# tsurumeso/vocal-remover

Hardware: NVIDIA H100
Metric: seconds-of-audio/sec separated (n_fft=2048, hop=1024) (higher is better)
Workload: dtype bf16x3 (split-bf16 operands hi+lo, 3 wgmma passes, fp32 accumulate); fft/lstm fp32

## Files before the change

### vocal-remover_b200/csrc/api.cu

```cuda
#include <stdio.h>
#include <string.h>

#include <string>

#include "../../include/vr_b200.h"
#include "engine.h"
#include "kernels.h"
#include "tc_plan.h"

struct vr_ctx {
  vr::Engine* eng;
  std::string err;
};

static std::string g_create_err;

static int fail(vr_ctx* c, const std::string& m) {
  (c ? c->err : g_create_err) = m;
  return -1;
}
static void use_device(const vr_ctx* c) {
  if (c && c->eng) cudaSetDevice(c->eng->cfg().device);
}
static int done(vr_ctx* c, bool ok) {
// ... 330 lines not shown
  if (e != cudaSuccess) return fail(ctx, std::string("vr_shared_alloc: cudaMalloc: ") + cudaGetErrorString(e));
  cudaIpcMemHandle_t h;
  e = cudaIpcGetMemHandle(&h, p);
  if (e != cudaSuccess) {
    cudaFree(p);
    return fail(ctx, std::string("vr_shared_alloc: cudaIpcGetMemHandle: ") + cudaGetErrorString(e));
  }
  memcpy(handle64, &h, 64);
  *dev_ptr = p;
  return 0;
}

int vr_shared_open(vr_ctx* ctx, const unsigned char* handle64, void** dev_ptr) {
  CHECK_CTX(ctx);
  if (!dev_ptr || !handle64) return fail(ctx, "vr_shared_open: bad arguments");
  cudaIpcMemHandle_t h;
  memcpy(&h, handle64, 64);
  void* p = nullptr;
  cudaError_t e = cudaIpcOpenMemHandle(&p, h, cudaIpcMemLazyEnablePeerAccess);
  if (e != cudaSuccess) return fail(ctx, std::string("vr_shared_open: cudaIpcOpenMemHandle: ") + cudaGetErrorString(e));
  *dev_ptr = p;
  return 0;
}

int vr_shared_close(vr_ctx* ctx, void* dev_ptr, int32_t owner) {
  CHECK_CTX(ctx);
  if (!dev_ptr) return 0;
  cudaError_t e = owner ? cudaFree(dev_ptr) : cudaIpcCloseMemHandle(dev_ptr);
  if (e != cudaSuccess) return fail(ctx, std::string("vr_shared_close: ") + cudaGetErrorString(e));
  return 0;
}

int64_t vr_launch_count(const vr_ctx* ctx) { return ctx && ctx->eng ? ctx->eng->launches : 0; }

int vr_profile_enable(vr_ctx* ctx, int32_t on) {
  CHECK_CTX(ctx);
  ctx->eng->profile_enable(on != 0);
  return 0;
}

int vr_profile_read(vr_ctx* ctx, double* out6) {
  CHECK_CTX(ctx);
  return done(ctx, ctx->eng->profile_read(out6));
}

int vr_profile_dump(vr_ctx* ctx, char* text, int64_t cap, int64_t* needed) {
  CHECK_CTX(ctx);
  std::string t;
  if (!ctx->eng->profile_dump(t)) return done(ctx, false);
  if (needed) *needed = (int64_t)t.size() + 1;
  if (text && cap > 0) {
    const size_t n = t.size() < (size_t)cap - 1 ? t.size() : (size_t)cap - 1;
    memcpy(text, t.data(), n);
    text[n] = 0;
  }
  return 0;
}

int vr_debug_conv(vr_ctx* ctx, const float* x, int32_t N, int32_t Cin, int32_t H, int32_t W, const float* w,
                  const float* bias, int32_t Cout, int32_t k, int32_t stride, int32_t dil_h, int32_t dil_w, int32_t act,
                  int32_t use_tc, float* y, void* stream) {
  CHECK_CTX(ctx);
  return done(ctx, ctx->eng->debug_conv(x, N, Cin, H, W, w, bias, Cout, k, stride, dil_h, dil_w, act, use_tc, y,
                                        (cudaStream_t)stream));
}

int vr_debug_decoder(vr_ctx* ctx, const float* low, int32_t N, int32_t Cl, int32_t h, int32_t w, const float* skip,
                     int32_t Cs, const float* wgt, const float* bias, int32_t Cout, int32_t act, int32_t fused, float* y,
                     void* stream) {
  CHECK_CTX(ctx);
  return done(ctx, ctx->eng->debug_decoder(low, N, Cl, h, w, skip, Cs, wgt, bias, Cout, act, fused, y,
                                           (cudaStream_t)stream));
}

int vr_debug_tensor(vr_ctx* ctx, const char* name, int32_t n0, int32_t n, float* out, int64_t* shape4, void* stream) {
  CHECK_NET(ctx);
  if (!name || !shape4) return fail(ctx, "vr_debug_tensor: name and shape4 are required");
  return done(ctx, ctx->eng->debug_tensor(name, n0, n, out, shape4, (cudaStream_t)stream));
}

int vr_debug_set(int32_t key, int32_t value) {
  int* knob = key == 0 ? &vr::g_debug.trace : key == 2 ? &vr::g_debug.rows_wide : key == 3 ? &vr::g_debug.halo
            : key == 6 ? &vr::g_debug.kskip : key == 7 ? &vr::g_debug.crop_mask
            : key == 8 ? &vr::g_debug.pair : key == 9 ? &vr::g_debug.pair_stores : nullptr;
  if (!knob) return -1;
  *knob = value;
  return 0;
}

int64_t vr_debug_trace(uint64_t* host_out, int64_t capacity) {
  return vr::tc_rows_read_trace((unsigned long long*)host_out, (long long)capacity);
}

}
```

### vocal-remover_b200/csrc/conv_tc_rows.cu

```cuda
#include <stdio.h>

#include "engine.h"
#include "tc_common.cuh"
#include "tc_plan.h"

namespace vr {

static constexpr int kInterpWarps = 10;
static constexpr int kConsumerWarps = 8;
static constexpr int kTmaWarp = kConsumerWarps;
static constexpr int kInterpWarp0 = kConsumerWarps + 1;
__host__ __device__ constexpr int rows_per_tile(int BN) { return BN == 64 ? 2 : BN == 32 ? 4 : 8; }
static constexpr int kUpProducerWarps = 12;
static constexpr int kUpConsumerRegs = 128;
static constexpr int kUpProducerRegs = 72;
static constexpr int kUpLaunchRegs = 96;
static_assert(kConsumerWarps * kUpConsumerRegs + kUpProducerWarps * kUpProducerRegs <=
                  (kConsumerWarps + kUpProducerWarps) * kUpLaunchRegs,
              "setmaxnreg.inc would wait forever for registers the block does not own");
__host__ __device__ constexpr int rows_threads(bool up) { return 32 * (kConsumerWarps + (up ? kUpProducerWarps : 1)); }
static constexpr int kRowPx = 130;
static constexpr int kBoxPx = 136;
static constexpr int kMaxASlots = 8;
static constexpr int kStaticSmem = 3072;
static constexpr int kSrcPx = 68;
static constexpr uint32_t kKB = 32;
static constexpr uint32_t kRowB = kKB * 2;
static constexpr uint32_t kAPlane = kBoxPx * kRowB;
static constexpr uint32_t kASlot = 2 * kAPlane;

static constexpr int kTraceEvents = 2048;
__device__ unsigned long long g_rows_trace[3 * kTraceEvents * 3];

template <int BN>
struct RowsGeom {
  static constexpr uint32_t kBPlane = 3 * BN * kRowB;
  static constexpr uint32_t kBKw = 2 * kBPlane;
  static constexpr uint32_t kBBuf = 3 * kBKw;
};

struct RowsParams {
  int N, H, W, tiles_w, tiles_h, n_tiles, total_tiles;
  int col0;
  int chunks, CinPadR, Cout, act;
  int n_aslots;
  bf16* out_hi;
  bf16* out_lo;
  int64_t osn, osh;
  int osw;
  int vec16;
  const float* bias;
  int up_chunks, xH, xW;
  const bf16* x_hi;
  const bf16* x_lo;
  int64_t xsn, xsh;
  int xsw;
  int trace;
  unsigned long long kmask;
  int a_c_off;
  int l_chunk;
  int n_uslots;
  float up_sh, up_sw;
  const float* dot_w;
  float* dot_out;
  MaskOutParams mask;
};

struct RowsTile {
  int nt, w0, h0, n;
};
template <int R>
__device__ __forceinline__ RowsTile rows_tile(const RowsParams& p, int tile) {
  RowsTile t;
  t.nt = tile % p.n_tiles;
  int mt = tile / p.n_tiles;
  t.w0 = p.col0 + (mt % p.tiles_w) * 128;
  mt /= p.tiles_w;
  t.h0 = (mt % p.tiles_h) * R;
  t.n = mt / p.tiles_h;
  return t;
}

struct RowsConsumer {
  MbarRing a_up, a_tma, b;
  HeldSlot held_b;
};

template <int BN, int R, int r>
__device__ __forceinline__ MbarRing consume_rows(MbarRing a, RowsConsumer& st, float* acc, uint32_t (&fr)[2][16],
                                                 uint32_t lrow, uint32_t bsrc, uint32_t dhi, uint32_t ksm, int lane) {
  constexpr int o_lo = r - 2 < 0 ? 0 : r - 2;
  constexpr int o_hi = r > R - 1 ? R - 1 : r;
  a.wait_full();
  const uint32_t row = lrow + (uint32_t)a.slot * kASlot;
#pragma unroll
  for (int kw = 0; kw < 3; ++kw) {
    uint32_t* f = fr[(3 * r + kw) & 1];
    const uint32_t q = (row >> 6) + (uint32_t)kw;
#pragma unroll
    for (int ks = 0; ks < 2; ++ks) {
      if (!((ksm >> ks) & 1u)) continue;
      const uint32_t a = (q << 6) + ((((uint32_t)(2 * ks) + ((uint32_t)lane >> 4)) ^ ((q >> 1) & 3u)) << 4);
      ldsm_x4(f + 8 * ks, a);
      ldsm_x4(f + 8 * ks + 4, a + kAPlane);
    }
    wg_fence();
#pragma unroll
    for (int ks = 0; ks < 2; ++ks) {
      if (!((ksm >> ks) & 1u)) continue;
      const uint32_t bo = (uint32_t)(kw * RowsGeom<BN>::kBKw + ks * 32) >> 4;
#pragma unroll
      for (int o = o_lo; o <= o_hi; ++o) {
        const uint32_t b_row = bsrc + (((uint32_t)((2 - (r - o)) * BN) * kRowB) >> 4) + bo;
        wgmma_split3_rs<BN>(acc + o * (BN / 2), f + 8 * ks, f + 8 * ks + 4, b_row,
                            b_row + (RowsGeom<BN>::kBPlane >> 4), dhi);
      }
    }
    wg_commit();
    if (kw == 2) warp_arrive(a.empty(), lane);
    wg_wait<1>();
    st.held_b.release(st.b, lane);
  }
  a.advance();
  if constexpr (r + 1 < R + 2)
    return consume_rows<BN, R, r + 1>(a, st, acc, fr, lrow, bsrc, dhi, ksm, lane);
  else
    return a;
}

__device__ __forceinline__ float dot_pair(float v0, float v1, const float* bias_s, const float* dot_s, int c, float slope) {
  const float t0 = v0 + bias_s[c], t1 = v1 + bias_s[c + 1];
  return fmaf(fmaxf(t0, 0.f) + slope * fminf(t0, 0.f), dot_s[c], (fmaxf(t1, 0.f) + slope * fminf(t1, 0.f)) * dot_s[c + 1]);
}

template <int BN>
__device__ __forceinline__ void mask_pixel(const RowsParams& p, const float* v, const float* bias_s,
                                           const float* mask_s, float slope, int lane, int n, int bin, int w) {
  float x[BN / 4];
#pragma unroll
  for (int j = 0; j < BN / 8; ++j) {
    const int c = 8 * j + 2 * (lane & 3);
    const float t0 = v[4 * j] + bias_s[c], t1 = v[4 * j + 1] + bias_s[c + 1];
    const float y0 = fmaxf(t0, 0.f) + slope * fminf(t0, 0.f);
    const float y1 = fmaxf(t1, 0.f) + slope * fminf(t1, 0.f);
    const float2 hf = bf2_to_f2(f2_to_bf2(y0, y1));
    const float2 lf = bf2_to_f2(f2_to_bf2(y0 - hf.x, y1 - hf.y));
    x[2 * j] = hf.x + lf.x;
    x[2 * j + 1] = hf.y + lf.y;
  }
  const float* wm = mask_s + (lane & 1) * BN;
  float a = 0.f;
#pragma unroll
  for (int c = 0; c < BN; ++c)
    a = fmaf(__shfl_sync(0xffffffffu, x[2 * (c >> 3) + (c & 1)], (lane & ~3) | ((c >> 1) & 3)), wm[c], a);
  const float m = 1.f / (1.f + expf(-a));
  const int tr = w - p.col0;
  const int64_t t = p.mask.t_base0 + (int64_t)n * p.mask.roi_t + tr;
  const bool nyquist = (lane & 2) != 0;
  if (t < 0 || t >= p.mask.t_limit || (nyquist && bin != p.H - 1)) return;
  float* d = p.mask.out + (int64_t)n * p.mask.stride_n + (int64_t)(nyquist ? bin + 1 : bin) * p.mask.stride_bin +
             p.mask.t_base0 + tr + ((lane & 1) ? p.mask.stride_c : 0);
  *d = p.mask.accumulate ? (*d + m) * 0.5f : m;
}

template <int BN, bool UP>
__global__ void __launch_bounds__(rows_threads(UP), 1)
    conv_tc_rows_kernel(const __grid_constant__ CUtensorMap tmA, const __grid_constant__ CUtensorMap tmB,
                        const __grid_constant__ CUtensorMap tmL, const RowsParams p) {
  typedef RowsGeom<BN> G;
  constexpr int R = rows_per_tile(BN);
  extern __shared__ uint8_t smem_raw[];
  __shared__ __align__(8) uint64_t bar_afull[kMaxASlots];
  __shared__ __align__(8) uint64_t bar_aempty[kMaxASlots];
  __shared__ __align__(8) uint64_t bar_bfull[2];
  __shared__ __align__(8) uint64_t bar_bempty[2];
  __shared__ float bias_s[256];
  __shared__ float dot_s[256];

  const int warp = __shfl_sync(0xffffffffu, (int)threadIdx.x >> 5, 0);
  const int lane = threadIdx.x & 31;
  const uint32_t smem_base = (smem_u32(smem_raw) + 1023u) & ~1023u;
  const uint32_t a_base = smem_base;
  const uint32_t b_base = smem_base + (uint32_t)p.n_aslots * kASlot;
  MbarRing a_up(smem_u32(&bar_afull[0]), smem_u32(&bar_aempty[0]), 0, p.n_uslots);
  MbarRing a_tma(smem_u32(&bar_afull[0]), smem_u32(&bar_aempty[0]), p.n_uslots, p.n_aslots);
  MbarRing b_ring(smem_u32(&bar_bfull[0]), smem_u32(&bar_bempty[0]), 0, 2);

  if (warp == kTmaWarp && lane == 0) {
    tma_prefetch(&tmA);
    tma_prefetch(&tmB);
    a_up.init(kInterpWarps, kConsumerWarps);
    a_tma.init(1, kConsumerWarps);
    b_ring.init(1, kConsumerWarps);
    asm volatile("fence.mbarrier_init.release.cluster;" ::: "memory");
  }
  for (int i = threadIdx.x; i < p.n_tiles * BN; i += blockDim.x) {
    bias_s[i] = __ldg(p.bias + i);
    dot_s[i] = p.dot_out && i < p.Cout ? __ldg(p.dot_w + i) : 0.f;
  }
  constexpr bool kMaskable = UP && BN <= 32;
  if constexpr (kMaskable) {
    if (p.mask.out)
      for (int i = threadIdx.x; i < 2 * BN; i += blockDim.x) dot_s[i] = __ldg(p.mask.w + i);
  }
  __syncthreads();
  if (warp < kConsumerWarps) {
    if constexpr (UP) setmaxnreg_inc<kUpConsumerRegs>();
    const int wg = warp >> 2;
    const float slope = act_slope(p.act);
    const uint32_t dhi = desc_hi(8 * kRowB, 2u);
    const uint32_t lrow = a_base + (uint32_t)(64 * wg + 16 * (warp & 3) + (lane & 15)) * kRowB;
    RowsConsumer st{a_up, a_tma, b_ring};
    float acc[R * BN / 2];
    uint32_t fr[2][16];
    for (int tile = blockIdx.x; tile < p.total_tiles; tile += gridDim.x) {
#pragma unroll
      for (int i = 0; i < R * BN / 2; ++i) acc[i] = 0.f;
      for (int cc = 0; cc < p.chunks; ++cc) {
        st.b.wait_full();
        const uint32_t bsrc = desc_lo(b_base + (uint32_t)st.b.slot * G::kBBuf);
        const bool up = cc < p.up_chunks;
        const uint32_t gm = chunk_groups(p.kmask, cc);
        const uint32_t ksm = ((gm & 0x3u) ? 1u : 0u) | ((gm & 0xCu) ? 2u : 0u);
        const MbarRing a = consume_rows<BN, R, 0>(up ? st.a_up : st.a_tma, st, acc, fr, lrow, bsrc, dhi, ksm, lane);
        st.a_up.slot = up ? a.slot : st.a_up.slot;
        st.a_up.phase = up ? a.phase : st.a_up.phase;
        st.a_tma.slot = up ? st.a_tma.slot : a.slot;
        st.a_tma.phase = up ? st.a_tma.phase : a.phase;
        st.held_b.hold(st.b);
        st.b.advance();
      }
      wg_wait<0>();
      st.held_b.release_last(st.b, lane);

      const RowsTile tl = rows_tile<R>(p, tile);
      const int w0 = tl.w0, h0 = tl.h0, n = tl.n;
      const int c_lane = tl.nt * BN + 2 * (lane & 3);
      auto dot = [&](const float* v, int orow, int px) {
        float d = 0.f;
#pragma unroll
        for (int j = 0; j < BN / 8; ++j) d += dot_pair(v[4 * j], v[4 * j + 1], bias_s, dot_s, c_lane + 8 * j, slope);
        d += __shfl_xor_sync(0xffffffffu, d, 1);
        d += __shfl_xor_sync(0xffffffffu, d, 2);
        if ((lane & 3) == 0) atomicAdd(p.dot_out + ((int64_t)n * p.H + (h0 + orow)) * p.W + (w0 + px), d);
      };
      const int px0 = 64 * wg + 16 * (warp & 3) + (lane >> 2);
#pragma unroll
      for (int orow = 0; orow < R; ++orow) {
        if constexpr (UP) {
          constexpr bool kPixel8 = BN > 16;
#pragma unroll
          for (int hr = 0; hr < 2; ++hr) {
            const int px = px0 + 8 * hr;
            const float* v = acc + orow * (BN / 2) + 2 * hr;
            if constexpr (kMaskable) {
              if (p.mask.out) {
                mask_pixel<BN>(p, v, bias_s, dot_s, slope, lane, n, h0 + orow, w0 + px);
                continue;
              }
            }
            if (p.dot_out) dot(v, orow, px);
            const int64_t obase = (int64_t)n * p.osn + (int64_t)(h0 + orow) * p.osh + (int64_t)(w0 + px) * p.osw;
            epilogue_pixel8<BN>(v, bias_s, tl.nt * BN, p.Cout, slope, lane, p.out_hi + obase, p.out_lo + obase,
                                kPixel8 && p.vec16 != 0);
          }
        } else {
          const float* v = acc + orow * (BN / 2);
          if (p.dot_out) {
            dot(v, orow, px0);
            dot(v + 2, orow, px0 + 8);
          }
          const int64_t obase = (int64_t)n * p.osn + (int64_t)(h0 + orow) * p.osh + (int64_t)(w0 + px0) * p.osw;
          const EpiDest d{p.out_hi, p.out_lo, {obase, obase + 8 * (int64_t)p.osw}, {true, true}, tl.nt * BN, p.Cout,
                          p.vec16 != 0};
          epilogue_store<BN>(v, bias_s, slope, lane, d);
        }
      }
    }
  } else {
    if constexpr (UP) setmaxnreg_dec<kUpProducerRegs>();
    if (warp == kTmaWarp) {
      if (elect_one_sync()) {
#ifdef VR_TRACE
        const bool tr = p.trace && blockIdx.x == 0;
#else
        constexpr bool tr = false;
#endif
        int tn = 0;
        for (int tile = blockIdx.x; tile < p.total_tiles; tile += gridDim.x) {
          const RowsTile tl = rows_tile<R>(p, tile);
          const int nt = tl.nt, w0 = tl.w0, h0 = tl.h0, n = tl.n;
          for (int cc = 0; cc < p.chunks; ++cc) {
            b_ring.wait_empty();
            const uint32_t bdst = b_base + (uint32_t)b_ring.slot * G::kBBuf;
            mbar_expect_tx(b_ring.full(), G::kBBuf);
#pragma unroll
            for (int kw = 0; kw < 3; ++kw)
              tma_load_3d(bdst + (uint32_t)kw * G::kBKw, &tmB, kw * p.CinPadR + cc * (int)kKB, nt * 3 * BN, 0,
                          b_ring.full());
            b_ring.advance();
            if (cc < p.up_chunks) continue;
            const bool from_l = cc == p.l_chunk;
            const int c0 = from_l ? 0 : cc * (int)kKB + p.a_c_off;
            for (int r = 0; r < R + 2; ++r) {
              const unsigned long long t0 = tr ? clock64() : 0ull;
              a_tma.wait_empty();
              mbar_expect_tx(a_tma.full(), kASlot);
              tma_load_5d(a_base + (uint32_t)a_tma.slot * kASlot, from_l ? &tmL : &tmA, c0, w0 - 1, h0 - 1 + r, n, 0,
                          a_tma.full());
              if (tr && tn < kTraceEvents) {
                g_rows_trace[(1 * kTraceEvents + tn) * 3 + 0] = t0;
                g_rows_trace[(1 * kTraceEvents + tn) * 3 + 1] = clock64();
                g_rows_trace[(1 * kTraceEvents + tn) * 3 + 2] = 0ull;
                ++tn;
              }
              a_tma.advance();
            }
          }
        }
      }
      __syncwarp();
    } else if (UP && warp < kInterpWarp0 + kInterpWarps) {
      if (p.up_chunks > 0) {
        const int wk = warp - kInterpWarp0;
        const int xi = lane >> 2, j = lane & 3;
        const int sx = 7 * wk + xi;
        const bool emit = xi < 7 && sx < kSrcPx;
        const float inv_sw = p.up_sw > 0.f ? 1.f / p.up_sw : 0.f;
#ifdef VR_TRACE
        const bool tr = p.trace && blockIdx.x == 0 && wk == 0;
#else
        constexpr bool tr = false;
#endif
        int tn = 0;
        const int my_tiles = (p.total_tiles - (int)blockIdx.x + (int)gridDim.x - 1) / (int)gridDim.x;
        const int fills = my_tiles * p.up_chunks * (R + 2);
        int f_tile = blockIdx.x, f_cc = 0, f_r = 0, f_h0 = 0, f_X = 0;
        int64_t f_base = 0;
        bool f_px = false;
        auto fetch_tile = [&]() {
          const RowsTile tl = rows_tile<R>(p, f_tile);
          f_h0 = tl.h0 - 1;
          f_X = (int)(p.up_sw * (tl.w0 > 0 ? tl.w0 - 1 : 0)) + sx;
          f_px = sx < kSrcPx && f_X < p.xW;
          f_base = (int64_t)tl.n * p.xsn + (int64_t)f_X * p.xsw + j * 8;
        };
        fetch_tile();
        bf16x8 qah, qch, qal, qcl, nah, nch, nal, ncl;
        float q_ly = 0.f, n_ly = 0.f;
        qah = qch = qal = qcl = nah = nch = nal = ncl = make_uint4(0, 0, 0, 0);
        auto fetch = [&]() {
          qah = nah; qch = nch; qal = nal; qcl = ncl;
          q_ly = n_ly;
          const int h = f_h0 + f_r;
          const bool grp = (chunk_groups(p.kmask, f_cc) >> j) & 1u;
          if (f_tile < p.total_tiles && h >= 0 && h < p.H && grp && f_px) {
            const float fy = p.up_sh * h;
            const int y0 = (int)fy;
            n_ly = fy - (float)y0;
            const int64_t o0 = f_base + (int64_t)y0 * p.xsh + f_cc * 32;
            const int64_t o1 = o0 + (y0 < p.xH - 1 ? p.xsh : 0);
// ... 98 lines not shown
            }
          }
        }
      }
      }
  }
}

#define VR_ROWS_FOR_ALL(X) X(16, true) X(16, false) X(32, true) X(32, false) X(64, true) X(64, false)

static int rows_b_bytes(int BN) {
#define VR_ROWS_B(BN_, UP_) if (BN == BN_) return (int)(2 * RowsGeom<BN_>::kBBuf);
  VR_ROWS_FOR_ALL(VR_ROWS_B)
#undef VR_ROWS_B
  return 0;
}

bool tc_rows_has(int BN) { return rows_b_bytes(BN) > 0; }

cudaError_t tc_rows_launch(const ConvLayer& L, TcConv& tc, const ActView& in, const ActView& out, cudaStream_t s,
                           std::string& err, const ConvFusion& f) {
  const ActView* up_src = f.up;
  if (up_src && (!tc.fuses_upsample(up_src->C) || up_src->H * 2 != in.H || up_src->W * 2 != in.W || up_src->sw % 8)) {
    err = "tc_rows_launch: fused upsample needs a half-resolution source of 32k channels";
    return cudaErrorInvalidValue;
  }
  if (up_src && up_src->C + in.C > tc.CinPad) {
    err = "tc_rows_launch: with a fused upsample the input must hold only the channels after the up-sampled ones";
    return cudaErrorInvalidValue;
  }
  const ActView* last = f.last_chunk;
  if (last && (last->H != in.H || last->W != in.W || last->N != in.N || last->C > tc.KB)) {
    err = "tc_rows_launch: the last-chunk tensor must match the input geometry and fit one chunk";
    return cudaErrorInvalidValue;
  }
  const CUtensorMap* map_a = tc_activation_map(tc, in, kBoxPx, 1, 1, 1, err, L.name);
  const CUtensorMap* map_l = last ? tc_activation_map(tc, *last, kBoxPx, 1, 1, 1, err, L.name) : map_a;
  if (!map_a || !map_l) return cudaErrorInvalidValue;
  if (f.mask && !tc.fuses_mask(L.Cout, f.mask->offset, up_src != nullptr)) {
    err = "tc_rows_launch: the fused output layer needs a fused upsample, one N tile of Cout <= 32 channels and a "
          "kept width that is a multiple of 128";
    return cudaErrorInvalidValue;
  }
  const int col0 = f.mask ? f.mask->offset : 0;
  RowsParams p;
  p.N = out.N; p.H = out.H; p.W = out.W;
  const bool up = up_src != nullptr;
  p.col0 = col0;
  p.tiles_w = (out.W - 2 * col0) / 128; p.tiles_h = out.H / rows_per_tile(tc.BN); p.n_tiles = tc.n_tiles;
  p.total_tiles = p.tiles_w * p.tiles_h * out.N * tc.n_tiles;
  p.chunks = tc.chunks; p.CinPadR = tc.CinPad; p.Cout = L.Cout; p.act = L.act;
  p.out_hi = out.hi; p.out_lo = out.lo;
  p.osn = out.sn; p.osh = out.sh; p.osw = out.sw;
  p.vec16 = tc_vec16(out);
  p.bias = tc.bias.get();
  p.up_chunks = 0; p.xH = p.xW = 0;
  p.x_hi = p.x_lo = nullptr; p.xsn = p.xsh = 0; p.xsw = 0;
  p.trace = g_debug.trace == 1 ? 1 : 0;
  p.up_sh = p.up_sw = 0.f;
  p.dot_w = f.dot_w; p.dot_out = f.dot_w ? f.dot_out : nullptr;
  p.mask = f.mask ? *f.mask : MaskOutParams{};
  p.a_c_off = 0;
  p.l_chunk = last ? tc.chunks - 1 : -1;
  p.kmask = g_debug.kskip == 1 ? tc.kmask : ~0ull;
  if (up_src) {
    p.a_c_off = -up_src->C;
    p.up_chunks = up_src->C / 32;
    p.xH = up_src->H; p.xW = up_src->W;
    p.x_hi = up_src->hi; p.x_lo = up_src->lo;
    p.xsn = up_src->sn; p.xsh = up_src->sh; p.xsw = up_src->sw;
    if ((reinterpret_cast<uintptr_t>(up_src->hi) | reinterpret_cast<uintptr_t>(up_src->lo)) & 15) {
      err = "tc_rows_launch: upsample source planes must be 16-byte aligned";
      return cudaErrorInvalidValue;
    }
    p.up_sh = in.H > 1 ? (float)(up_src->H - 1) / (float)(in.H - 1) : 0.f;
    p.up_sw = in.W > 1 ? (float)(up_src->W - 1) / (float)(in.W - 1) : 0.f;
  }
  const TcDevice& dv = tc_device();
  if (!dv.ok) {
    err = "tc_rows_launch: cannot query the current device";
    return cudaErrorInvalidValue;
  }
  const int b_bytes = rows_b_bytes(tc.BN);
  p.n_aslots = (dv.max_smem - kStaticSmem - 1024 - b_bytes) / (int)kASlot;
  if (p.n_aslots > kMaxASlots) p.n_aslots = kMaxASlots;
  if (p.n_aslots < (p.up_chunks > 0 ? 4 : 2)) {
    err = "tc_rows_launch: shared memory too small";
    return cudaErrorInvalidValue;
  }
  p.n_uslots = p.up_chunks > 0 ? p.n_aslots - p.n_aslots / 2 : 0;
  if (p.up_chunks > 0 && p.n_aslots - p.n_uslots < 2) p.n_uslots = p.n_aslots - 2;
  const int dyn = p.n_aslots * (int)kASlot + b_bytes + 1024;
  const int grid = p.total_tiles < dv.num_sms ? p.total_tiles : dv.num_sms;
  const int threads = rows_threads(up);
#define VR_ROWS_LAUNCH(BN_, UP_)                                                              \
  if (tc.BN == BN_ && up == UP_) {                                                            \
    conv_tc_rows_kernel<BN_, UP_><<<grid, threads, dyn, s>>>(*map_a, tc.map_b, *map_l, p);    \
    return cudaGetLastError();                                                                \
  }
  VR_ROWS_FOR_ALL(VR_ROWS_LAUNCH)
#undef VR_ROWS_LAUNCH
  err = "tc_rows_launch: no kernel instantiation for this channel tile";
  return cudaErrorInvalidValue;
}


int tc_rows_read_trace(unsigned long long* out, long long capacity) {
  const long long n = 3LL * kTraceEvents * 3;
  if (capacity < n) return -1;
  if (cudaMemcpyFromSymbol(out, g_rows_trace, sizeof(unsigned long long) * (size_t)n) != cudaSuccess) return -1;
  return (int)n;
}

void tc_rows_set_attributes(int max_smem) {
#define VR_ROWS_SET(BN_, UP_)                                                                        \
  cudaFuncSetAttribute(conv_tc_rows_kernel<BN_, UP_>, cudaFuncAttributeMaxDynamicSharedMemorySize,   \
                       max_smem - kStaticSmem);                                                      \
  cudaFuncSetAttribute(conv_tc_rows_kernel<BN_, UP_>, cudaFuncAttributePreferredSharedMemoryCarveout, 100);
  VR_ROWS_FOR_ALL(VR_ROWS_SET)
#undef VR_ROWS_SET
}

}
```

### vocal-remover_b200/csrc/tc_common.cuh

```cuda
#pragma once
#include <cuda.h>
#include <stdint.h>
#include <stdio.h>

#include "common.cuh"

namespace vr {

__device__ __forceinline__ uint32_t smem_u32(const void* p) { return (uint32_t)__cvta_generic_to_shared(p); }

__device__ __forceinline__ bool elect_one_sync() {
  uint32_t pred;
  asm volatile(
      "{\n\t"
      ".reg .pred P1;\n\t"
      "elect.sync _|P1, 0xffffffff;\n\t"
      "selp.u32 %0, 1, 0, P1;\n\t"
      "}"
      : "=r"(pred));
  return pred != 0;
}

__device__ __forceinline__ void mbar_init(uint32_t bar, uint32_t count) {
  asm volatile("mbarrier.init.shared::cta.b64 [%0], %1;" ::"r"(bar), "r"(count));
// ... 21 lines not shown
      "WAIT_DONE:\n\t"
      "}" ::"r"(bar),
      "r"(parity)
      : "memory");
#else
  asm volatile(
      "{\n\t"
      ".reg .pred p;\n\t"
      "WAIT_LOOP:\n\t"
      "mbarrier.try_wait.parity.shared::cta.b64 p, [%0], %1;\n\t"
      "@p bra WAIT_DONE;\n\t"
      "bra WAIT_LOOP;\n\t"
      "WAIT_DONE:\n\t"
      "}" ::"r"(bar),
      "r"(parity)
      : "memory");
#endif
}
__device__ __forceinline__ void warp_arrive(uint32_t bar, int lane) {
  __syncwarp();
  if (lane == 0) mbar_arrive(bar);
}

struct MbarRing {
  uint32_t full0, empty0;
  int lo, hi, slot;
  uint32_t phase;

  __device__ __forceinline__ MbarRing(uint32_t full0_, uint32_t empty0_, int lo_, int hi_)
      : full0(full0_), empty0(empty0_), lo(lo_), hi(hi_), slot(lo_), phase(0) {}
  __device__ __forceinline__ uint32_t full(int s) const { return full0 + (uint32_t)s * 8u; }
  __device__ __forceinline__ uint32_t empty(int s) const { return empty0 + (uint32_t)s * 8u; }
  __device__ __forceinline__ uint32_t full() const { return full(slot); }
  __device__ __forceinline__ uint32_t empty() const { return empty(slot); }
  __device__ __forceinline__ void wait_full() const { mbar_wait(full(), phase); }
  __device__ __forceinline__ void wait_empty() const { mbar_wait(empty(), phase ^ 1u); }
  __device__ __forceinline__ void advance() {
    if (++slot == hi) {
      slot = lo;
      phase ^= 1u;
    }
  }
  __device__ __forceinline__ void init(uint32_t full_count, uint32_t empty_count) const {
    for (int s = lo; s < hi; ++s) {
      mbar_init(full(s), full_count);
      mbar_init(empty(s), empty_count);
    }
  }
};

struct HeldSlot {
  int slot = -1;
  __device__ __forceinline__ void hold(const MbarRing& r) { slot = r.slot; }
  __device__ __forceinline__ void release(const MbarRing& r, int lane) {
    if (slot >= 0) {
      warp_arrive(r.empty(slot), lane);
      slot = -1;
    }
  }
  __device__ __forceinline__ void release_last(const MbarRing& r, int lane) {
    warp_arrive(r.empty(slot), lane);
    slot = -1;
  }
};

__device__ __forceinline__ void tma_prefetch(const CUtensorMap* map) {
  asm volatile("prefetch.tensormap [%0];" ::"l"(map) : "memory");
}
__device__ __forceinline__ void tma_load_5d(uint32_t dst, const CUtensorMap* map, int c0, int c1, int c2, int c3,
                                            int c4, uint32_t bar) {
  asm volatile(
      "cp.async.bulk.tensor.5d.shared::cluster.global.tile.mbarrier::complete_tx::bytes [%0], [%1, {%2, %3, %4, %5, "
      "%6}], [%7];" ::"r"(dst),
      "l"(map), "r"(c0), "r"(c1), "r"(c2), "r"(c3), "r"(c4), "r"(bar)
      : "memory");
}
__device__ __forceinline__ void tma_load_3d(uint32_t dst, const CUtensorMap* map, int c0, int c1, int c2,
                                            uint32_t bar) {
  asm volatile(
      "cp.async.bulk.tensor.3d.shared::cluster.global.tile.mbarrier::complete_tx::bytes [%0], [%1, {%2, %3, %4}], "
      "[%5];" ::"r"(dst),
      "l"(map), "r"(c0), "r"(c1), "r"(c2), "r"(bar)
      : "memory");
}

__device__ __forceinline__ uint32_t desc_lo(uint32_t addr) { return ((addr & 0x3FFFFu) >> 4) | (1u << 16); }
__device__ __forceinline__ uint32_t desc_hi(uint32_t sbo_bytes, uint32_t layout_type) {
  return (sbo_bytes >> 4) | (layout_type << 30);
}
__device__ __forceinline__ uint64_t desc64(uint32_t lo, uint32_t hi) { return ((uint64_t)hi << 32) | lo; }

__device__ __forceinline__ void wg_fence() { asm volatile("wgmma.fence.sync.aligned;" ::: "memory"); }
__device__ __forceinline__ void wg_commit() { asm volatile("wgmma.commit_group.sync.aligned;" ::: "memory"); }
template <int PENDING>
__device__ __forceinline__ void wg_wait() {
  asm volatile("wgmma.wait_group.sync.aligned %0;" ::"n"(PENDING) : "memory");
}

template <int N>
struct Wgmma;
template <>
struct Wgmma<16> {
  static __device__ __forceinline__ void mma(float* d, uint64_t a, uint64_t b) {
    asm volatile(
        "wgmma.mma_async.sync.aligned.m64n16k16.f32.bf16.bf16 {%0, %1, %2, %3, %4, %5, %6, %7}, %8, %9, 1, 1, 1, 0, 0;"
        : "+f"(d[0]), "+f"(d[1]), "+f"(d[2]), "+f"(d[3]), "+f"(d[4]), "+f"(d[5]), "+f"(d[6]), "+f"(d[7])
        : "l"(a), "l"(b)
        : "memory");
  }
};
template <>
struct Wgmma<32> {
  static __device__ __forceinline__ void mma(float* d, uint64_t a, uint64_t b) {
    asm volatile(
        "wgmma.mma_async.sync.aligned.m64n32k16.f32.bf16.bf16 {%0, %1, %2, %3, %4, %5, %6, %7, %8, %9, %10, %11, %12, %13, %14, %15}, %16, %17, 1, 1, 1, 0, 0;"
        : "+f"(d[0]), "+f"(d[1]), "+f"(d[2]), "+f"(d[3]), "+f"(d[4]), "+f"(d[5]), "+f"(d[6]), "+f"(d[7]), "+f"(d[8]), "+f"(d[9]), "+f"(d[10]), "+f"(d[11]), "+f"(d[12]), "+f"(d[13]), "+f"(d[14]), "+f"(d[15])
        : "l"(a), "l"(b)
        : "memory");
  }
};
template <>
struct Wgmma<48> {
  static __device__ __forceinline__ void mma(float* d, uint64_t a, uint64_t b) {
    asm volatile(
        "wgmma.mma_async.sync.aligned.m64n48k16.f32.bf16.bf16 {%0, %1, %2, %3, %4, %5, %6, %7, %8, %9, %10, %11, %12, %13, %14, %15, %16, %17, %18, %19, %20, %21, %22, %23}, %24, %25, 1, 1, 1, 0, 0;"
        : "+f"(d[0]), "+f"(d[1]), "+f"(d[2]), "+f"(d[3]), "+f"(d[4]), "+f"(d[5]), "+f"(d[6]), "+f"(d[7]), "+f"(d[8]), "+f"(d[9]), "+f"(d[10]), "+f"(d[11]), "+f"(d[12]), "+f"(d[13]), "+f"(d[14]), "+f"(d[15]), "+f"(d[16]), "+f"(d[17]), "+f"(d[18]), "+f"(d[19]), "+f"(d[20]), "+f"(d[21]), "+f"(d[22]), "+f"(d[23])
        : "l"(a), "l"(b)
        : "memory");
  }
};
template <>
struct Wgmma<64> {
  static __device__ __forceinline__ void mma(float* d, uint64_t a, uint64_t b) {
    asm volatile(
        "wgmma.mma_async.sync.aligned.m64n64k16.f32.bf16.bf16 {%0, %1, %2, %3, %4, %5, %6, %7, %8, %9, %10, %11, %12, %13, %14, %15, %16, %17, %18, %19, %20, %21, %22, %23, %24, %25, %26, %27, %28, %29, %30, %31}, %32, %33, 1, 1, 1, 0, 0;"
        : "+f"(d[0]), "+f"(d[1]), "+f"(d[2]), "+f"(d[3]), "+f"(d[4]), "+f"(d[5]), "+f"(d[6]), "+f"(d[7]), "+f"(d[8]), "+f"(d[9]), "+f"(d[10]), "+f"(d[11]), "+f"(d[12]), "+f"(d[13]), "+f"(d[14]), "+f"(d[15]), "+f"(d[16]), "+f"(d[17]), "+f"(d[18]), "+f"(d[19]), "+f"(d[20]), "+f"(d[21]), "+f"(d[22]), "+f"(d[23]), "+f"(d[24]), "+f"(d[25]), "+f"(d[26]), "+f"(d[27]), "+f"(d[28]), "+f"(d[29]), "+f"(d[30]), "+f"(d[31])
        : "l"(a), "l"(b)
        : "memory");
  }
};
template <>
struct Wgmma<80> {
  static __device__ __forceinline__ void mma(float* d, uint64_t a, uint64_t b) {
    asm volatile(
        "wgmma.mma_async.sync.aligned.m64n80k16.f32.bf16.bf16 {%0, %1, %2, %3, %4, %5, %6, %7, %8, %9, %10, %11, %12, %13, %14, %15, %16, %17, %18, %19, %20, %21, %22, %23, %24, %25, %26, %27, %28, %29, %30, %31, %32, %33, %34, %35, %36, %37, %38, %39}, %40, %41, 1, 1, 1, 0, 0;"
        : "+f"(d[0]), "+f"(d[1]), "+f"(d[2]), "+f"(d[3]), "+f"(d[4]), "+f"(d[5]), "+f"(d[6]), "+f"(d[7]), "+f"(d[8]), "+f"(d[9]), "+f"(d[10]), "+f"(d[11]), "+f"(d[12]), "+f"(d[13]), "+f"(d[14]), "+f"(d[15]), "+f"(d[16]), "+f"(d[17]), "+f"(d[18]), "+f"(d[19]), "+f"(d[20]), "+f"(d[21]), "+f"(d[22]), "+f"(d[23]), "+f"(d[24]), "+f"(d[25]), "+f"(d[26]), "+f"(d[27]), "+f"(d[28]), "+f"(d[29]), "+f"(d[30]), "+f"(d[31]), "+f"(d[32]), "+f"(d[33]), "+f"(d[34]), "+f"(d[35]), "+f"(d[36]), "+f"(d[37]), "+f"(d[38]), "+f"(d[39])
        : "l"(a), "l"(b)
        : "memory");
  }
};
template <>
struct Wgmma<96> {
  static __device__ __forceinline__ void mma(float* d, uint64_t a, uint64_t b) {
    asm volatile(
        "wgmma.mma_async.sync.aligned.m64n96k16.f32.bf16.bf16 {%0, %1, %2, %3, %4, %5, %6, %7, %8, %9, %10, %11, %12, %13, %14, %15, %16, %17, %18, %19, %20, %21, %22, %23, %24, %25, %26, %27, %28, %29, %30, %31, %32, %33, %34, %35, %36, %37, %38, %39, %40, %41, %42, %43, %44, %45, %46, %47}, %48, %49, 1, 1, 1, 0, 0;"
        : "+f"(d[0]), "+f"(d[1]), "+f"(d[2]), "+f"(d[3]), "+f"(d[4]), "+f"(d[5]), "+f"(d[6]), "+f"(d[7]), "+f"(d[8]), "+f"(d[9]), "+f"(d[10]), "+f"(d[11]), "+f"(d[12]), "+f"(d[13]), "+f"(d[14]), "+f"(d[15]), "+f"(d[16]), "+f"(d[17]), "+f"(d[18]), "+f"(d[19]), "+f"(d[20]), "+f"(d[21]), "+f"(d[22]), "+f"(d[23]), "+f"(d[24]), "+f"(d[25]), "+f"(d[26]), "+f"(d[27]), "+f"(d[28]), "+f"(d[29]), "+f"(d[30]), "+f"(d[31]), "+f"(d[32]), "+f"(d[33]), "+f"(d[34]), "+f"(d[35]), "+f"(d[36]), "+f"(d[37]), "+f"(d[38]), "+f"(d[39]), "+f"(d[40]), "+f"(d[41]), "+f"(d[42]), "+f"(d[43]), "+f"(d[44]), "+f"(d[45]), "+f"(d[46]), "+f"(d[47])
        : "l"(a), "l"(b)
        : "memory");
  }
};
template <>
struct Wgmma<112> {
  static __device__ __forceinline__ void mma(float* d, uint64_t a, uint64_t b) {
    asm volatile(
        "wgmma.mma_async.sync.aligned.m64n112k16.f32.bf16.bf16 {%0, %1, %2, %3, %4, %5, %6, %7, %8, %9, %10, %11, %12, %13, %14, %15, %16, %17, %18, %19, %20, %21, %22, %23, %24, %25, %26, %27, %28, %29, %30, %31, %32, %33, %34, %35, %36, %37, %38, %39, %40, %41, %42, %43, %44, %45, %46, %47, %48, %49, %50, %51, %52, %53, %54, %55}, %56, %57, 1, 1, 1, 0, 0;"
        : "+f"(d[0]), "+f"(d[1]), "+f"(d[2]), "+f"(d[3]), "+f"(d[4]), "+f"(d[5]), "+f"(d[6]), "+f"(d[7]), "+f"(d[8]), "+f"(d[9]), "+f"(d[10]), "+f"(d[11]), "+f"(d[12]), "+f"(d[13]), "+f"(d[14]), "+f"(d[15]), "+f"(d[16]), "+f"(d[17]), "+f"(d[18]), "+f"(d[19]), "+f"(d[20]), "+f"(d[21]), "+f"(d[22]), "+f"(d[23]), "+f"(d[24]), "+f"(d[25]), "+f"(d[26]), "+f"(d[27]), "+f"(d[28]), "+f"(d[29]), "+f"(d[30]), "+f"(d[31]), "+f"(d[32]), "+f"(d[33]), "+f"(d[34]), "+f"(d[35]), "+f"(d[36]), "+f"(d[37]), "+f"(d[38]), "+f"(d[39]), "+f"(d[40]), "+f"(d[41]), "+f"(d[42]), "+f"(d[43]), "+f"(d[44]), "+f"(d[45]), "+f"(d[46]), "+f"(d[47]), "+f"(d[48]), "+f"(d[49]), "+f"(d[50]), "+f"(d[51]), "+f"(d[52]), "+f"(d[53]), "+f"(d[54]), "+f"(d[55])
// ... 253 lines not shown
```

### vocal-remover_b200/csrc/tc_plan.h

```cpp
#pragma once
#include <cuda.h>

#include <map>
#include <tuple>

#include "engine.h"

namespace vr {

enum TcKind {
  TC_NONE,
  TC_GENERIC,
  TC_ROWS,
  TC_HALO,
};

enum TcPair { PAIR_NONE = 0, PAIR_M = 1, PAIR_N = 2 };

typedef std::tuple<const void*, const void*, int, int, int, int, int, int, int, int> ViewKey;

struct TcConv {
  TcKind kind = TC_NONE;
  int H = 0, W = 0;
  int KB = 0, CinPad = 0, chunks = 0, BN = 0, n_tiles = 0;
  unsigned long long kmask = ~0ull;
  DevPtr<bf16> w_planes;
  DevPtr<float> bias;
  CUtensorMap map_b;
  std::map<ViewKey, CUtensorMap> map_a;
  TcPair pair = PAIR_NONE;
  int pair_KB = 0;
  CUtensorMap map_b_pair;
  bool fuses_upsample(int up_C) const { return kind == TC_ROWS && up_C % 32 == 0 && up_C <= CinPad; }
  bool fuses_dot() const { return kind == TC_ROWS; }
  bool fuses_mask(int Cout, int offset, bool up) const {
    const int kept = W - 2 * offset;
    return kind == TC_ROWS && up && n_tiles == 1 && BN <= 32 && BN == Cout && offset >= 0 && kept > 0 &&
           kept % 128 == 0;
  }
};

TcKind tc_choose(const ConvLayer& L, int H, int W, bool rows_wide);
const CUtensorMap* tc_activation_map(TcConv& tc, const ActView& v, int bw, int bh, int bn, int es, std::string& err,
                                     const std::string& name, int kb = 0);

cudaError_t tc_rows_launch(const ConvLayer& L, TcConv& tc, const ActView& in, const ActView& out, cudaStream_t s,
                           std::string& err, const ConvFusion& f);
void tc_rows_set_attributes(int max_smem);
bool tc_rows_has(int BN);
int tc_rows_read_trace(unsigned long long* out, long long capacity);

cudaError_t tc_halo_launch(const ConvLayer& L, TcConv& tc, const ActView& in, const ActView& out, cudaStream_t s,
                           std::string& err);
void tc_halo_set_attributes(int max_smem);
bool tc_halo_has(int BN);

struct TcDevice {
  bool ok = false;
  int num_sms = 0, max_smem = 0;
};
const TcDevice& tc_device();

struct TcDebug {
  int trace = 0;
  int rows_wide = 0;
  int halo = 0;
  int kskip = 1;
  int crop_mask = 1;
  int pair = 0;
  int pair_stores = 0;
};
extern TcDebug g_debug;

bool tc_vec16(const ActView& out);

}
```

Baseline: 3079.

## Stage row-kernel epilogue outputs in shared memory and write them with TMA stores

For row-conv kernels with BN<=32, consumer warps now write the activated hi/lo bf16 outputs into a swizzled, double-buffered shared-memory staging area. Per output row, each warpgroup fences, syncs on a named barrier and issues a 5D TMA bulk store, replacing scattered per-thread global stores. This costs some shared memory, which can reduce the number of A pipeline slots, and adds a per-row named barrier. The path is on by default when the output layout allows it and no mask fusion is used, and a debug knob selects the old register epilogue for A/B profiling.

```diff
diff --git a/profiles/row_epilogue.py b/profiles/row_epilogue.py
--- /dev/null
+++ b/profiles/row_epilogue.py
@@ -0,0 +1,132 @@
+import argparse
+import collections
+import ctypes
+import json
+import os
+import re
+import statistics
+import subprocess
+import sys
+
+ROOT = os.path.dirname(os.path.dirname(os.path.abspath(__file__)))
+PKG = os.path.join(ROOT, 'vocal-remover_b200')
+for p in (ROOT, PKG):
+    if p not in sys.path:
+        sys.path.insert(0, p)
+
+
+def _gpu_info():
+    try:
+        r = subprocess.run(['nvidia-smi', '--query-gpu=name,power.limit,clocks.max.sm,clocks.sm',
+                            '--format=csv,noheader'], capture_output=True, text=True, timeout=30)
+        name, power, max_clock, clock = [s.strip() for s in r.stdout.splitlines()[0].split(',')]
+        return dict(gpu=name, power_limit=power, max_sm_clock=max_clock, sm_clock=clock)
+    except Exception as e:
+        return dict(gpu=None, nvidia_smi_error=str(e))
+
+
+ROW_LAYER = re.compile(r'\.(enc1|enc2\.conv2|dec2\.conv1|dec1\.conv1)(\+\w+)*$')
+
+
+def _profiled_step(ctx, step):
+    ctx.check(ctx.lib.vr_profile_enable(ctx.handle, 1), 'vr_profile_enable')
+    step()
+    need = ctypes.c_int64(0)
+    ctx.check(ctx.lib.vr_profile_dump(ctx.handle, None, 0, ctypes.byref(need)), 'vr_profile_dump')
+    buf = ctypes.create_string_buffer(need.value)
+    ctx.check(ctx.lib.vr_profile_dump(ctx.handle, buf, need.value, None), 'vr_profile_dump')
+    ctx.check(ctx.lib.vr_profile_enable(ctx.handle, 0), 'vr_profile_enable')
+    out = collections.OrderedDict()
+    for ln in buf.value.decode().splitlines():
+        name, n, h, w, tc, ms, _ = ln.split()
+        if int(tc) != 1 or not ROW_LAYER.search(name):
+            continue
+        key = (name, int(h), int(w))
+        a = out.setdefault(key, [0, 0.0])
+        a[0] += int(n)
+        a[1] += float(ms)
+    return out
+
+
+def _out_channels(state_dict):
+    return {name: t.shape[0] for name, t in state_dict.items() if name.endswith('weight') and t.dim() == 4}
+
+
+def _cout(couts, layer):
+    layer = layer.split('+')[0]
+    for name, c in couts.items():
+        if name.startswith(layer + '.'):
+            return c
+    return None
+
+
+def main():
+    ap = argparse.ArgumentParser()
+    ap.add_argument('--rounds', type=int, default=3)
+    ap.add_argument('--warmup', type=int, default=2)
+    ap.add_argument('--seconds', type=float, default=240.0)
+    ap.add_argument('--batch', type=int, default=27)
+    ap.add_argument('--out', type=str, default='')
+    args = ap.parse_args()
+    import torch
+    import inference
+    from lib import _native, nets, synth
+    assert torch.cuda.is_available(), 'this profile needs a GPU'
+    dev = torch.device('cuda:0')
+    info = _gpu_info()
+    model = nets.CascadedNet(2048, 1024, 32, 128)
+    state = synth.to_torch_state_dict(synth.make_state_dict())
+    model.load_state_dict(state)
+    model.to(dev)
+    sp = inference.Separator(model, dev, args.batch, 256, False)
+    wave = torch.from_numpy(synth.sine_mix(args.seconds)).to(dev)
+    ctx = sp._ctx()
+    lib = _native.load_library()
+    couts = _out_channels(state)
+
+    def step():
+        sp.separate_wave(wave)
+        torch.cuda.synchronize()
+
+    times = {0: collections.defaultdict(list), 1: collections.defaultdict(list)}
+    counts = {}
+    try:
+        for key in (0, 1):
+            assert lib.vr_debug_set(10, key) == 0
+            for _ in range(args.warmup):
+                step()
+        for _ in range(args.rounds):
+            for key in (0, 1):
+                assert lib.vr_debug_set(10, key) == 0
+                for k, (n, ms) in _profiled_step(ctx, step).items():
+                    times[key][k].append(ms)
+                    counts[k] = n
+    finally:
+        lib.vr_debug_set(10, 0)
+    info_end = _gpu_info()
+    rows = []
+    for k in times[0]:
+        name, h, w = k
+        c = _cout(couts, name)
+        rows.append(dict(layer=name, H=h, W=w, images=counts[k], cout=c,
+                         out_bytes=counts[k] * h * w * c * 4 if c else None,
+                         ms_staged=statistics.median(times[0][k]), ms_register=statistics.median(times[1][k])))
+    print('%s, power limit %s, max SM clock %s, SM clock at start %s / end %s' % (
+        info.get('gpu'), info.get('power_limit'), info.get('max_sm_clock'), info.get('sm_clock'),
+        info_end.get('sm_clock')))
+    print('%-34s %5s %5s %6s %9s %9s %9s %6s' % ('layer', 'H', 'W', 'Cout', 'out MB', 'ms TMA', 'ms reg', 'gain'))
+    for r in rows:
+        print('%-34s %5d %5d %6s %9s %9.3f %9.3f %5.1f%%' % (
+            r['layer'], r['H'], r['W'], r['cout'] or '-', '%.1f' % (r['out_bytes'] / 1e6) if r['out_bytes'] else '-',
+            r['ms_staged'], r['ms_register'],
+            100.0 * (1.0 - r['ms_staged'] / r['ms_register']) if r['ms_register'] else 0.0))
+    t0, t1 = sum(r['ms_staged'] for r in rows), sum(r['ms_register'] for r in rows)
+    print('row-kernel layers: %.2f ms with staged TMA stores, %.2f ms with the register epilogue' % (t0, t1))
+    if args.out:
+        with open(args.out, 'w') as f:
+            json.dump(dict(gpu=info, sm_clock_end=info_end.get('sm_clock'), rounds=args.rounds, rows=rows), f,
+                      indent=1)
+
+
+if __name__ == '__main__':
+    main()
diff --git a/vocal-remover_b200/csrc/api.cu b/vocal-remover_b200/csrc/api.cu
--- a/vocal-remover_b200/csrc/api.cu
+++ b/vocal-remover_b200/csrc/api.cu
@@ -436,7 +436,8 @@
 int vr_debug_set(int32_t key, int32_t value) {
   int* knob = key == 0 ? &vr::g_debug.trace : key == 2 ? &vr::g_debug.rows_wide : key == 3 ? &vr::g_debug.halo
             : key == 6 ? &vr::g_debug.kskip : key == 7 ? &vr::g_debug.crop_mask
-            : key == 8 ? &vr::g_debug.pair : key == 9 ? &vr::g_debug.pair_stores : nullptr;
+            : key == 8 ? &vr::g_debug.pair : key == 9 ? &vr::g_debug.pair_stores
+            : key == 10 ? &vr::g_debug.rows_stores : nullptr;
   if (!knob) return -1;
   *knob = value;
   return 0;
diff --git a/vocal-remover_b200/csrc/conv_tc_rows.cu b/vocal-remover_b200/csrc/conv_tc_rows.cu
--- a/vocal-remover_b200/csrc/conv_tc_rows.cu
+++ b/vocal-remover_b200/csrc/conv_tc_rows.cu
@@ -49,6 +49,7 @@
   int64_t osn, osh;
   int osw;
   int vec16;
+  int staged;
   const float* bias;
   int up_chunks, xH, xW;
   const bf16* x_hi;
@@ -66,6 +67,36 @@
   MaskOutParams mask;
 };
 
+__host__ __device__ constexpr int rows_stage_buf(int BN) { return BN <= 32 ? 2 * 64 * 2 * BN : 0; }
+__host__ __device__ constexpr int rows_stage_bytes(int BN) { return 4 * rows_stage_buf(BN); }
+
+template <int BN>
+__device__ __forceinline__ void stage_pixel(const float* v, const float* bias_s, int c0, float slope, int lane,
+                                            uint32_t buf, int px) {
+  constexpr uint32_t kRow = 2 * BN, kPlane = 64 * kRow;
+  const uint32_t q = (uint32_t)lane & 3u;
+  const uint32_t swz = ((uint32_t)px * kRow >> 7) & (uint32_t)(BN / 8 - 1);
+#pragma unroll
+  for (int j = 0; j < BN / 8; ++j) {
+    uint32_t hi, lo;
+    act_split2(v[4 * j], v[4 * j + 1], bias_s, c0 + 8 * j + 2 * (int)q, slope, hi, lo);
+    const uint32_t a = buf + (uint32_t)px * kRow + ((((uint32_t)j) ^ swz) << 4) + 4u * q;
+    st_shared_u32(a, hi);
+    st_shared_u32(a + kPlane, lo);
+  }
+}
+
+__device__ __forceinline__ void stage_commit(const CUtensorMap* tmO, uint32_t buf, bool issuer, int wg, int c0, int w,
+                                             int h, int n) {
+  fence_proxy_async_smem();
+  if (issuer) bulk_wait_read<0>();
+  named_bar_sync(1 + wg, 128);
+  if (issuer) {
+    tma_store_5d(tmO, buf, c0, w, h, n, 0);
+    bulk_commit();
+  }
+}
+
 struct RowsTile {
   int nt, w0, h0, n;
 };
@@ -166,7 +197,8 @@
 template <int BN, bool UP>
 __global__ void __launch_bounds__(rows_threads(UP), 1)
     conv_tc_rows_kernel(const __grid_constant__ CUtensorMap tmA, const __grid_constant__ CUtensorMap tmB,
-                        const __grid_constant__ CUtensorMap tmL, const RowsParams p) {
+                        const __grid_constant__ CUtensorMap tmL, const __grid_constant__ CUtensorMap tmO,
+                        const RowsParams p) {
   typedef RowsGeom<BN> G;
   constexpr int R = rows_per_tile(BN);
   extern __shared__ uint8_t smem_raw[];
@@ -182,6 +214,7 @@
   const uint32_t smem_base = (smem_u32(smem_raw) + 1023u) & ~1023u;
   const uint32_t a_base = smem_base;
   const uint32_t b_base = smem_base + (uint32_t)p.n_aslots * kASlot;
+  const uint32_t stage_base = b_base + (uint32_t)(2 * G::kBBuf);
   MbarRing a_up(smem_u32(&bar_afull[0]), smem_u32(&bar_aempty[0]), 0, p.n_uslots);
   MbarRing a_tma(smem_u32(&bar_afull[0]), smem_u32(&bar_aempty[0]), p.n_uslots, p.n_aslots);
   MbarRing b_ring(smem_u32(&bar_bfull[0]), smem_u32(&bar_bempty[0]), 0, 2);
@@ -189,6 +222,7 @@
   if (warp == kTmaWarp && lane == 0) {
     tma_prefetch(&tmA);
     tma_prefetch(&tmB);
+    if (p.staged) tma_prefetch(&tmO);
     a_up.init(kInterpWarps, kConsumerWarps);
     a_tma.init(1, kConsumerWarps);
     b_ring.init(1, kConsumerWarps);
@@ -211,6 +245,9 @@
     const uint32_t dhi = desc_hi(8 * kRowB, 2u);
     const uint32_t lrow = a_base + (uint32_t)(64 * wg + 16 * (warp & 3) + (lane & 15)) * kRowB;
     RowsConsumer st{a_up, a_tma, b_ring};
+    constexpr bool kStaged = rows_stage_buf(BN) > 0;
+    const bool staged = kStaged && p.staged;
+    const bool issuer = (threadIdx.x & 127) == 0;
     float acc[R * BN / 2];
     uint32_t fr[2][16];
     for (int tile = blockIdx.x; tile < p.total_tiles; tile += gridDim.x) {
@@ -249,6 +286,7 @@
       for (int orow = 0; orow < R; ++orow) {
         if constexpr (UP) {
           constexpr bool kPixel8 = BN > 16;
+          const uint32_t buf = stage_base + (uint32_t)((2 * wg + (orow & 1)) * rows_stage_buf(BN));
 #pragma unroll
           for (int hr = 0; hr < 2; ++hr) {
             const int px = px0 + 8 * hr;
@@ -260,15 +298,33 @@
               }
             }
             if (p.dot_out) dot(v, orow, px);
+            if constexpr (kStaged) {
+              if (staged) {
+                stage_pixel<BN>(v, bias_s, tl.nt * BN, slope, lane, buf, px - 64 * wg);
+                continue;
+              }
+            }
             const int64_t obase = (int64_t)n * p.osn + (int64_t)(h0 + orow) * p.osh + (int64_t)(w0 + px) * p.osw;
             epilogue_pixel8<BN>(v, bias_s, tl.nt * BN, p.Cout, slope, lane, p.out_hi + obase, p.out_lo + obase,
                                 kPixel8 && p.vec16 != 0);
+          }
+          if constexpr (kStaged) {
+            if (staged) stage_commit(&tmO, buf, issuer, wg, tl.nt * BN, w0 + 64 * wg, h0 + orow, n);
           }
         } else {
           const float* v = acc + orow * (BN / 2);
           if (p.dot_out) {
             dot(v, orow, px0);
             dot(v + 2, orow, px0 + 8);
+          }
+          if constexpr (kStaged) {
+            if (staged) {
+              const uint32_t buf = stage_base + (uint32_t)((2 * wg + (orow & 1)) * rows_stage_buf(BN));
+              stage_pixel<BN>(v, bias_s, tl.nt * BN, slope, lane, buf, px0 - 64 * wg);
+              stage_pixel<BN>(v + 2, bias_s, tl.nt * BN, slope, lane, buf, px0 + 8 - 64 * wg);
+              stage_commit(&tmO, buf, issuer, wg, tl.nt * BN, w0 + 64 * wg, h0 + orow, n);
+              continue;
+            }
           }
           const int64_t obase = (int64_t)n * p.osn + (int64_t)(h0 + orow) * p.osh + (int64_t)(w0 + px0) * p.osw;
           const EpiDest d{p.out_hi, p.out_lo, {obase, obase + 8 * (int64_t)p.osw}, {true, true}, tl.nt * BN, p.Cout,
@@ -277,6 +333,7 @@
         }
       }
     }
+    if (staged && issuer) bulk_wait<0>();
   } else {
     if constexpr (UP) setmaxnreg_dec<kUpProducerRegs>();
     if (warp == kTmaWarp) {
@@ -541,20 +598,34 @@
     return cudaErrorInvalidValue;
   }
   const int b_bytes = rows_b_bytes(tc.BN);
-  p.n_aslots = (dv.max_smem - kStaticSmem - 1024 - b_bytes) / (int)kASlot;
-  if (p.n_aslots > kMaxASlots) p.n_aslots = kMaxASlots;
-  if (p.n_aslots < (p.up_chunks > 0 ? 4 : 2)) {
+  const int min_aslots = p.up_chunks > 0 ? 4 : 2;
+  auto aslots = [&](int stage_bytes) {
+    const int n = (dv.max_smem - kStaticSmem - 1024 - b_bytes - stage_bytes) / (int)kASlot;
+    return n > kMaxASlots ? kMaxASlots : n;
+  };
+  const int stage_bytes = rows_stage_bytes(tc.BN);
+  p.staged = stage_bytes > 0 && !f.mask && g_debug.rows_stores != 1 && tc_vec16(out) && out.lo > out.hi &&
+             aslots(stage_bytes) >= min_aslots;
+  p.n_aslots = aslots(p.staged ? stage_bytes : 0);
+  if (p.n_aslots < min_aslots) {
     err = "tc_rows_launch: shared memory too small";
     return cudaErrorInvalidValue;
   }
+  const CUtensorMap* map_o = map_a;
+  if (p.staged) {
+    ActView o = out;
+    o.C = L.Cout;
+    map_o = tc_activation_map(tc, o, 64, 1, 1, 1, err, L.name, tc.BN);
+    if (!map_o) return cudaErrorInvalidValue;
+  }
   p.n_uslots = p.up_chunks > 0 ? p.n_aslots - p.n_aslots / 2 : 0;
   if (p.up_chunks > 0 && p.n_aslots - p.n_uslots < 2) p.n_uslots = p.n_aslots - 2;
-  const int dyn = p.n_aslots * (int)kASlot + b_bytes + 1024;
+  const int dyn = p.n_aslots * (int)kASlot + b_bytes + (p.staged ? stage_bytes : 0) + 1024;
   const int grid = p.total_tiles < dv.num_sms ? p.total_tiles : dv.num_sms;
   const int threads = rows_threads(up);
 #define VR_ROWS_LAUNCH(BN_, UP_)                                                              \
   if (tc.BN == BN_ && up == UP_) {                                                            \
-    conv_tc_rows_kernel<BN_, UP_><<<grid, threads, dyn, s>>>(*map_a, tc.map_b, *map_l, p);    \
+    conv_tc_rows_kernel<BN_, UP_><<<grid, threads, dyn, s>>>(*map_a, tc.map_b, *map_l, *map_o, p); \
     return cudaGetLastError();                                                                \
   }
   VR_ROWS_FOR_ALL(VR_ROWS_LAUNCH)
diff --git a/vocal-remover_b200/csrc/tc_common.cuh b/vocal-remover_b200/csrc/tc_common.cuh
--- a/vocal-remover_b200/csrc/tc_common.cuh
+++ b/vocal-remover_b200/csrc/tc_common.cuh
@@ -127,6 +127,32 @@
       "[%5];" ::"r"(dst),
       "l"(map), "r"(c0), "r"(c1), "r"(c2), "r"(bar)
       : "memory");
+}
+
+__device__ __forceinline__ void tma_store_5d(const CUtensorMap* map, uint32_t src, int c0, int c1, int c2, int c3,
+                                             int c4) {
+  asm volatile(
+      "cp.async.bulk.tensor.5d.global.shared::cta.bulk_group [%0, {%2, %3, %4, %5, %6}], [%1];" ::"l"(map),
+      "r"(src), "r"(c0), "r"(c1), "r"(c2), "r"(c3), "r"(c4)
+      : "memory");
+}
+__device__ __forceinline__ void bulk_commit() { asm volatile("cp.async.bulk.commit_group;" ::: "memory"); }
+template <int N>
+__device__ __forceinline__ void bulk_wait_read() {
+  asm volatile("cp.async.bulk.wait_group.read %0;" ::"n"(N) : "memory");
+}
+template <int N>
+__device__ __forceinline__ void bulk_wait() {
+  asm volatile("cp.async.bulk.wait_group %0;" ::"n"(N) : "memory");
+}
+__device__ __forceinline__ void fence_proxy_async_smem() {
+  asm volatile("fence.proxy.async.shared::cta;" ::: "memory");
+}
+__device__ __forceinline__ void named_bar_sync(int id, int count) {
+  asm volatile("bar.sync %0, %1;" ::"r"(id), "r"(count) : "memory");
+}
+__device__ __forceinline__ void st_shared_u32(uint32_t addr, uint32_t v) {
+  asm volatile("st.shared.u32 [%0], %1;" ::"r"(addr), "r"(v) : "memory");
 }
 
 __device__ __forceinline__ uint32_t desc_lo(uint32_t addr) { return ((addr & 0x3FFFFu) >> 4) | (1u << 16); }
diff --git a/vocal-remover_b200/csrc/tc_plan.h b/vocal-remover_b200/csrc/tc_plan.h
--- a/vocal-remover_b200/csrc/tc_plan.h
+++ b/vocal-remover_b200/csrc/tc_plan.h
@@ -69,6 +69,7 @@
   int crop_mask = 1;
   int pair = 0;
   int pair_stores = 0;
+  int rows_stores = 0;
 };
 extern TcDebug g_debug;
 
```

After: 3115, median of 6. +1.1%, better.
